# neggles/neurosis

Hardware: AMD Instinct MI355X
Metric: train images/sec (node) SDXL 1024^2 (higher is better)
Workload: dtype bf16

## Files before the change

include/neurosis_hip.h:

```cpp
#ifndef NEUROSIS_HIP_H
#define NEUROSIS_HIP_H

#ifdef __cplusplus
extern "C" {
#endif

const char* nk_last_error(void);
int nk_abi_version(void);

int nk_linear_fwd(const void* x, const void* w, const float* bias, const void* residual, void* y,
                  int M, int N, int K, long ldx, long ldw, long ldr, long ldy, float alpha, void* stream);
int nk_linear_dgrad(const void* dy, const void* w, const void* dx_add, void* dx, int M, int N, int K,
                    long lddy, long ldw, long ldadd, long lddx, void* stream);
long nk_linear_fwd_geglu_ok(int M, int I, int K);
int nk_linear_fwd_geglu(const void* x, const void* w, const float* bias, void* u, void* h, int M, int I, int K, long ldx, long ldw, long ldu,
                        long ldh, void* stream);
int nk_linear_dgrad_geglu(const void* dy, const void* w, const void* u, void* du, int M, int N, int I, long lddy, long ldw, long ldu,
                          long lddu, void* stream);
int nk_linear_fwd_geglu_s(const void* x, const void* w, const float* bias, void* s, void* h, int M, int I, int K, long ldx, long ldw, long lds,
                          long ldh, void* stream);
int nk_linear_dgrad_geglu_s(const void* dy, const void* w, const void* s, void* du, int M, int N, int I, long lddy, long ldw, long lds,
                            long lddu, void* stream);
int nk_linear_wgrad(const void* dy, const void* x, float* dw, int M, int N, int K, long lddy, long ldx,
                    long lddw, int accumulate, void* stream);
// ... 15 lines not shown

int nk_linear_fwd_batched(const void* const* x, const void* const* w, void* const* y, int count, int M, int N, int K,
                          long ldx, long ldw, long ldy, void* stream);

int nk_linear_wgrad_batched(const void* const* dy, const void* const* x, float* const* dw, float* const* dbias, int count, int M, int N,
                            int K, long lddy, long ldx, long lddw, int accumulate, void* stream);

typedef struct NkConvDesc {
  int N, H, W, Cin;
  int Cout, KH, KW;
  int stride;
  int pad_t, pad_l;
  int Ho, Wo;
  int upsample;
} NkConvDesc;
int nk_conv2d_fwd(const NkConvDesc* d, const void* x, const void* w, const float* bias, const void* rowvec,
                  const void* residual, void* y, void* stream);
long nk_conv2d_stats_tiles(const NkConvDesc* d, int stats_groups);
int nk_conv2d_fwd_stats(const NkConvDesc* d, const void* x, const void* w, const float* bias, const void* rowvec, const void* residual,
                        void* y, float* stats_part, int stats_groups, void* stream);
int nk_conv3x3_few_channels_fwd(const void* x, const void* w, const float* bias, void* y, int N, int H, int W, int Cout, int cin_real,
                                void* stream);
int nk_conv_weight_flip(const void* w, void* wt, int Cout, int Cin, int taps, void* stream);
long nk_conv2d_dgrad_flipped_ok(const NkConvDesc* d);
int nk_conv2d_dgrad_flipped(const NkConvDesc* d, const void* dy, const void* wt, void* dx, void* stream);
int nk_conv2d_dgrad(const NkConvDesc* d, const void* dy, const void* w, void* dx, void* stream);
int nk_conv2d_wgrad(const NkConvDesc* d, const void* dy, const void* x, float* dw, int accumulate, void* stream);
int nk_conv2d_wgrad_bias(const NkConvDesc* d, const void* dy, const void* x, float* dw, float* dbias, int accumulate, void* stream);

typedef struct NkAttnDesc {
// ... 229 lines not shown
```

neurosis_amd/csrc/elementwise.hip:

```cpp
#include "../../include/neurosis_hip.h"
#include "nk_common.h"
#include "nk_ew.h"
#include "nk_reduce.h"
#include "norm_plan.h"

struct GegluFwd {
  const bf16_t* u; bf16_t* y; int I;
  __device__ void operator()(long, long row, int ch) const {
    float a[8], g[8];
    ew_load(u + row * 2 * I + ch * 8, a);
    ew_load(u + row * 2 * I + I + ch * 8, g);
#pragma unroll
    for (int e = 0; e < 8; ++e) a[e] *= gelu_erf(g[e]);
    ew_store(y + row * I + ch * 8, a);
  }
};
struct GegluBwd {
  const bf16_t *dy, *u; bf16_t* du; int I;
  __device__ void operator()(long, long row, int ch) const {
    float a[8], g[8], d[8], da[8], dg[8];
    ew_load(u + row * 2 * I + ch * 8, a);
    ew_load(u + row * 2 * I + I + ch * 8, g);
    ew_load(dy + row * I + ch * 8, d);
#pragma unroll
// ... 419 lines not shown
  const int tflip = taps - 1 - tap;
#pragma unroll
  for (int it = 0; it < 2; ++it) {
    const int idx = tid + 256 * it;
    const int r = idx >> 3, ch = idx & 7;
    if (ci0 + r < Cin && co0 + ch * 8 < Cout)
      *(uint4_t*)(wt + ((long)(ci0 + r) * taps + tflip) * Cout + co0 + ch * 8) = *(const uint4_t*)&tile[r][ch * 8];
  }
}
extern "C" int nk_conv_weight_flip(const void* w, void* wt, int Cout, int Cin, int taps, void* stream) {
  NK_CHECK_ARG(w && wt && Cout > 0 && Cin > 0 && taps > 0 && taps <= 65535);
  NK_CHECK_ARG((Cout & 7) == 0 && (Cin & 7) == 0);
  hipLaunchKernelGGL(conv_weight_flip_kernel, dim3((Cin + 63) / 64, (Cout + 63) / 64, taps), dim3(256), 0, (hipStream_t)stream, (const bf16_t*)w, (bf16_t*)wt,
                     Cout, Cin, taps);
  return nk_check_launch("conv_weight_flip_kernel");
}

__global__ __launch_bounds__(256) void conv3x3_few_channels_kernel(const bf16_t* __restrict__ x, const bf16_t* __restrict__ w, const float* __restrict__ bias,
                                                                   bf16_t* __restrict__ y, int N, int H, int W, int Cout, int groups_per_wave) {
  const int lane = threadIdx.x & 63, wave = threadIdx.x >> 6;
  const int r = lane & 15, g = lane >> 4;
  const int co_base = blockIdx.y * 128;
  bf16x8_t wf[8][2];
#pragma unroll
  for (int b = 0; b < 8; ++b) {
    const int co = co_base + b * 16 + r;
    uint2_t t0 = {0u, 0u}, t1 = {0u, 0u}, t8 = {0u, 0u};
    if (co < Cout) {
      t0 = *(const uint2_t*)(w + ((long)co * 9 + 2 * g) * 8);
      t1 = *(const uint2_t*)(w + ((long)co * 9 + 2 * g + 1) * 8);
// ... 508 lines not shown
```

neurosis_amd/csrc/gemm.hip:

```cpp
#include "nk_common.h"
#include "nk_gemm.h"
#include "gemm_plan.h"

#define NTHREADS 256
#define KC_IMAGE_BYTES (128 * 128)
#define MC_ROW_BYTES (128 * 2 + 16)
#define MC_IMAGE_BYTES (BK * MC_ROW_BYTES)
#define OPND_BYTES MC_IMAGE_BYTES
#define STAGE_BYTES (2 * OPND_BYTES)
#define SMEM_BYTES (2 * STAGE_BYTES)

static_assert(SMEM_BYTES >= BM * CS_LD * 4, "epilogue staging must fit");

__device__ __forceinline__ bool is_kc(int mode) { return mode == OP_KC || mode == OP_KCG; }

__device__ __forceinline__ long gather_offset(const NkGather& g, int n, int bh, int bw, int kh, int kw,
                                              int c, bool& valid) {
  int hn = bh + kh * g.ks;
  int wn = bw + kw * g.ks;
  bool ok = (hn >= 0) & (wn >= 0);
  ok &= (((hn | wn) & g.need_even) == 0);
  const int sh = g.div >> 1;
  int h = hn >> sh, w = wn >> sh;
  ok &= (h < g.H) & (w < g.W);
// ... 94 lines not shown
        float v = cs[row * CS_LD + col] * p.alpha;
        float* dst = C + (long)m * p.ldc + n;
        if (p.accumulate) unsafeAtomicAdd(dst, v);
        else *dst = v;
      }
    }
  } else {
    bf16_t* C = (bf16_t*)(p.nbatch ? p.Cb[blockIdx.z] : p.C);
    const bool vec = (p.N & 7) == 0;
#pragma unroll 2
    for (int it = 0; it < (TBM * BN / 8) / TNT; ++it) {
      int idx = tid + it * TNT;
      int row = idx >> 4, cc = idx & 15;
      int m = m0 + row, n = n0 + cc * 8;
      if (m >= p.M || n >= p.N) continue;
      float v[8];
      const float4_t c0 = *(const float4_t*)(cs + row * CS_LD + cc * 8);
      const float4_t c1 = *(const float4_t*)(cs + row * CS_LD + cc * 8 + 4);
      v[0] = c0[0]; v[1] = c0[1]; v[2] = c0[2]; v[3] = c0[3];
      v[4] = c1[0]; v[5] = c1[1]; v[6] = c1[2]; v[7] = c1[3];
      if (p.alpha != 1.0f) {
#pragma unroll
        for (int e = 0; e < 8; ++e) v[e] *= p.alpha;
      }
      if (vec) {
        if (p.bias) {
          const float4_t b0 = *(const float4_t*)(p.bias + n);
          const float4_t b1 = *(const float4_t*)(p.bias + n + 4);
          v[0] += b0[0]; v[1] += b0[1]; v[2] += b0[2]; v[3] += b0[3];
          v[4] += b1[0]; v[5] += b1[1]; v[6] += b1[2]; v[7] += b1[3];
        }
        if (p.rowvec) {
          unsigned b = fdiv((unsigned)m, p.fRowsPerBatch);
          float t[8];
          unpack8(*(const uint4_t*)(p.rowvec + (long)b * p.ld_rowvec + n), t);
#pragma unroll
          for (int e = 0; e < 8; ++e) v[e] += t[e];
        }
        if (p.residual) {
          float t[8];
          unpack8(*(const uint4_t*)(p.residual + (long)m * p.ldr + n), t);
#pragma unroll
          for (int e = 0; e < 8; ++e) v[e] += t[e];
        }
        *(uint4_t*)(C + (long)m * p.ldc + n) = pack8(v);
      } else {
        for (int e = 0; e < 8 && n + e < p.N; ++e) {
          float x = v[e];
          if (p.bias) x += p.bias[n + e];
          if (p.rowvec) x += bf2f(p.rowvec[(long)fdiv((unsigned)m, p.fRowsPerBatch) * p.ld_rowvec + n + e]);
          if (p.residual) x += bf2f(p.residual[(long)m * p.ldr + n + e]);
          C[(long)m * p.ldc + n + e] = f2bf(x);
        }
      }
    }
  }
}

__device__ __attribute__((aligned(64))) unsigned int nk_zero_page[16];

typedef __attribute__((address_space(1))) const void* nk_gptr;
typedef __attribute__((address_space(3))) void* nk_lptr;

__device__ __forceinline__ int mc_swz(int k) { return ((k & 3) | (((k >> 3) & 1) << 2)) << 1; }

template <int MODE, int NP = 4>
struct OperandDMA {
  const bf16_t* P;
  long ld;
  int R, r0, wave, lane;
  int pn[NP], pbh[NP], pbw[NP];
  int tkh0, tkh1, tkw0, tkw1, tc0, tc1;
  bool rvalid[NP < 2 ? 2 : NP];

  __device__ __forceinline__ int kc_row(int i) const { return wave * (NP * 8) + i * 8 + (lane >> 3); }
  __device__ __forceinline__ int kc_chunk() const { return (lane & 7) ^ (lane >> 3); }
  __device__ __forceinline__ int mc_k(int i) const { return (wave * NP + i) * 4 + (lane >> 4); }
  __device__ __forceinline__ int mc_var(int i) const { return (((wave * NP + i) * 4) >> 3) & 1; }
  __device__ __forceinline__ bool mc_valid(int v) const { return v ? rvalid[1] : rvalid[0]; }
  __device__ __forceinline__ int sel(int a0, int a1, int v) const { return v ? a1 : a0; }
  __device__ __forceinline__ int mc_chunk(int v) const { return (lane & 15) ^ (((lane >> 4) | (v << 2)) << 1); }

  __device__ __forceinline__ void init(const bf16_t* p, long ld_, int R_, int r0_, int tid, const NkGather& g) {
    P = p; ld = ld_; R = R_; r0 = r0_; wave = tid >> 6; lane = tid & 63;
    if constexpr (MODE == OP_KC || MODE == OP_KCG) {
#pragma unroll
      for (int i = 0; i < NP; ++i) {
        int r = r0 + kc_row(i);
        rvalid[i] = r < R;
        if constexpr (MODE == OP_KCG) {
          unsigned p_ = rvalid[i] ? (unsigned)r : 0u;
          unsigned n = fdiv(p_, g.fHoWo);
          unsigned rem = p_ - n * g.fHoWo.d;
          unsigned ph = fdiv(rem, g.fWo);
          unsigned pw = rem - ph * g.fWo.d;
          pn[i] = (int)n;
          pbh[i] = (int)ph * g.rs + g.off_h;
          pbw[i] = (int)pw * g.rs + g.off_w;
          if (g.div == 1 && (g.C & 63) == 0) pn[i] = ((pn[i] * g.H + pbh[i]) * g.W + pbw[i]) * g.C + kc_chunk() * 8;
        }
      }
    } else {
#pragma unroll
      for (int v = 0; v < 2; ++v) {
        int r = r0 + mc_chunk(v) * 8;
        rvalid[v] = r < R;
        if constexpr (MODE == OP_MCG) {
          unsigned rr = rvalid[v] ? (unsigned)r : 0u;
          unsigned tap = fdiv(rr, g.fC);
          const int c_ = (int)(rr - tap * g.fC.d);
          unsigned kh = fdiv(tap, g.fKW);
          const int kw_ = (int)(tap - kh * g.fKW.d);
          if (v == 0) { tc0 = c_; tkh0 = (int)kh; tkw0 = kw_; }
// ... 257 lines not shown
  const int per_group = GMv * ntn;
  const int group = wg / per_group;
  const int first_m = group * GMv;
  const int gm = min(GMv, ntm - first_m);
  const int in_group = wg - group * per_group;
  const int nt = in_group / gm;
  const int mt = first_m + (in_group - nt * gm);
  const int m0 = mt * BM, n0 = nt * BN;

  const int kbeg = blockIdx.y * p.ksplit_len;
  const int kend = min(p.K, kbeg + p.ksplit_len);
  const int nk = (kend - kbeg + BK - 1) / BK;

  OperandDMA<AMODE, NP> opa;
  OperandDMA<BMODE, NP> opb;
  opa.init(p.nbatch ? p.Ab[blockIdx.z] : p.A, p.lda, p.M, m0, tid, p.ga);
  opb.init(p.nbatch ? p.Bb[blockIdx.z] : p.B, p.ldb, p.N, n0, tid, p.gb);

  float4_t acc[4][NJ];
#pragma unroll
  for (int i = 0; i < 4; ++i)
#pragma unroll
    for (int j = 0; j < NJ; ++j) acc[i][j] = (float4_t){0.f, 0.f, 0.f, 0.f};
  constexpr bool CAN_BIAS = AMODE == OP_MC && OUT_F32 == 1;
  constexpr int NWN = NW == 4 ? 2 : 4, BPW = 4 / NWN;
  float* const dbias = CAN_BIAS ? (p.nbatch ? p.dbias_b[blockIdx.z] : p.dbias) : nullptr;
  const bool do_bias = CAN_BIAS && dbias != nullptr && nt == 0;
  const int wn_s = __builtin_amdgcn_readfirstlane(wn);
  float4_t accb[BPW];
#pragma unroll
  for (int u = 0; u < BPW; ++u) accb[u] = (float4_t){0.f, 0.f, 0.f, 0.f};
// ... 982 lines not shown
  if (amode == OP_MC) NK_CHECK_ARG((p.M & 7) == 0 && (p.lda & 7) == 0);
  if (bmode == OP_MC) NK_CHECK_ARG((p.N & 7) == 0 && (p.ldb & 7) == 0);
  if (bmode == OP_MCT) NK_CHECK_ARG((p.N & 7) == 0 && (p.tw.co_stride & 7) == 0 && (p.tw.tap_stride & 7) == 0);
  if (bmode == OP_MCG) NK_CHECK_ARG((p.gb.C & 7) == 0);
  if (p.residual) NK_CHECK_ARG(((uintptr_t)p.residual & 15) == 0 && ((p.ldr & 7) == 0 || (p.N & 7) != 0));
  if (!out_f32) NK_CHECK_ARG((p.ldc & 7) == 0 || (p.N & 7) != 0);
  if (p.fRowsPerBatch.d == 0) p.fRowsPerBatch = make_fastdiv(1);

  if (p.dbias || (p.nbatch && p.dbias_b[0])) NK_CHECK_ARG(amode == OP_MC && out_f32);
  if (p.geglu_h) {
    NK_CHECK_ARG(amode == OP_KC && bmode == OP_KC && !out_f32 && !p.nbatch && (p.N & 255) == 0 && (p.ld_h & 7) == 0 && !p.rowvec && !p.residual && p.alpha == 1.0f);
    NK_CHECK_ARG(((uintptr_t)p.geglu_h & 15) == 0 && (!p.bias || ((uintptr_t)p.bias & 15) == 0));
  } else if (p.geglu_u) {
    NK_CHECK_ARG(amode == OP_KC && bmode == OP_MC && !out_f32 && !p.nbatch && (p.N & 7) == 0 && (p.ld_u & 7) == 0 && !p.bias && !p.rowvec && !p.residual);
  }

  const TileEnv env = tile_env();
  const NkGemmPlan pl = nk_gemm_plan(p, amode, bmode, out_f32, allow_splitk, env);
  if (pl.err) {
    nk_set_error(__FILE__, __LINE__, pl.err);
    return NK_ERR_ARG;
  }
  if (pl.zero_c) NK_CHECK_ARG(p.ldc == p.N);
  const int logging = nk_launch_log_mode();
  char line[192];
  if (logging) nk_plan_line(pl, line, sizeof(line));
  if (logging == 3) {
    nk_launch_log_add(pl.name, line);
    return NK_OK;
  }
// ... 54 lines not shown
```

neurosis_amd/csrc/gemm_plan.h:

```cpp
#pragma once
#include "nk_gemm.h"
#include <stdio.h>
#include <stdlib.h>

enum { OP_KC = 0, OP_KCG = 1, OP_MC = 2, OP_MCT = 3, OP_MCG = 4 };

#define BM 128
#define BN 128
#define BK 64
#define GROUP_M 8
#define CS_LD 132
#define V2_OPND_BYTES 16384
#define V2_STAGE_BYTES (2 * V2_OPND_BYTES)
#define V2_SMEM_BYTES (BM * CS_LD * 4)
#define RING_NS 4
#define RING_SMEM_BYTES (RING_NS * V2_STAGE_BYTES)
#define SK_NT 512
#define SK_SMEM_BYTES (2 * V2_STAGE_BYTES)
#define SK_MAX_GRID 512
#define R64_NS 8
#define R64_OPND 8192
#define R64_STAGE (2 * R64_OPND)
#define R64_SMEM (R64_NS * R64_STAGE)
#define XL_BM 256
// ... 302 lines not shown

  if (p.geglu_h) {
    if (amode != OP_KC || !use_xl(env, p, amode, bmode, out_f32, 1)) {
      pl.err = "fused GEGLU forward on a shape the 256 x 256 kernel does not take (ask nk_linear_fwd_geglu_ok first)";
      return pl;
    }
    plan_split(pl, p, 1);
    plan_xl(pl, env, p, OP_KC);
    return pl;
  }
  if (p.geglu_u) {
    plan_split(pl, p, 1);
    plan_ring_or_dma(pl, env, p);
    return pl;
  }
  if (use_halo(env, p, amode, bmode, out_f32)) {
    const NkGather& g = p.ga;
    pl.bn = halo_bn(p.N); pl.halo_rows = halo_tile_rows(p); pl.flag = p.stats_part != nullptr;
    pl.tiles_per_image = cdiv(g.W, CH_TW) * cdiv(g.H, pl.halo_rows);
    plan_kernel(pl, NK_FAM_HALO, halo_name(pl.bn, pl.halo_rows, pl.flag), (long)p.halo_nb * pl.tiles_per_image * (p.N / pl.bn), 1, 1,
                halo_threads(pl.bn), halo_smem(pl.bn, pl.halo_rows));
    pl.k_rotate = k_rotate_on(env, g.C);
    return pl;
  }
  if (use_wgrad_halo(env, p, amode, bmode, out_f32)) {
    int per = 0;
    const int S = wgrad_halo_splits(p, per);
    const long nblk = (long)((p.M + WH_BCO - 1) / WH_BCO) * (p.gb.C / WH_BCI);
    pl.flag = p.dbias != nullptr;
    plan_kernel(pl, NK_FAM_WGRAD_HALO, pl.flag ? "nk_conv3x3_wgrad_halo_kernel<bias=1>" : "nk_conv3x3_wgrad_halo_kernel<bias=0>", nblk * S, 1, 1, 512, WH_SMEM);
// ... 61 lines not shown
```

neurosis_amd/csrc/nk_gemm.h:

```cpp
#pragma once
#include "nk_common.h"

struct NkGather {
  int H, W, C;
  int Ho, Wo;
  int KW;
  int rs, ks;
  int off_h, off_w;
  int div;
  int need_even;
  FastDiv fWo, fHoWo, fC, fKW;
};

struct NkTapW {
  long co_stride, tap_stride;
  FastDiv fCout;
};

struct NkGemmParams {
  const bf16_t* A;
  const bf16_t* B;
  long lda, ldb;
  int M, N, K;
  NkGather ga, gb;
// ... 18 lines not shown
  const bf16_t* Bb[8];
  void* Cb[8];
  unsigned* sk_flags;
  float* sk_ws;
  unsigned* sk_health;
  float* dbias;
  float* dbias_b[8];
  const bf16_t* geglu_u;
  long ld_u;
  bf16_t* geglu_h;
  long ld_h;
  int geglu_save;
  int halo_nb;
  float* stats_part;
  int stats_groups;
};
#define NK_MAX_BATCH 8

enum { NK_OP_KC = 0, NK_OP_KCG = 1, NK_OP_MC = 2, NK_OP_MCT = 3, NK_OP_MCG = 4 };

int nk_gemm_dispatch(NkGemmParams& p, int amode, int bmode, int out_f32, int allow_splitk, hipStream_t stream);
int nk_halo_tiles_per_image(const NkGemmParams& p, int* bn);
int nk_geglu_fwd_fusable(const NkGemmParams& p);
```

neurosis_amd/csrc/ops_gemm.hip:

```cpp
#include "../../include/neurosis_hip.h"
#include "nk_gemm.h"
#include <string.h>

static NkGemmParams zero_params() {
  NkGemmParams p;
  memset(&p, 0, sizeof(p));
  p.alpha = 1.0f;
  p.fRowsPerBatch = make_fastdiv(1);
  p.ga.fWo = p.ga.fHoWo = p.ga.fC = p.ga.fKW = make_fastdiv(1);
  p.gb.fWo = p.gb.fHoWo = p.gb.fC = p.gb.fKW = make_fastdiv(1);
  p.tw.fCout = make_fastdiv(1);
  return p;
}

extern "C" int nk_linear_fwd(const void* x, const void* w, const float* bias, const void* residual, void* y,
                             int M, int N, int K, long ldx, long ldw, long ldr, long ldy, float alpha,
                             void* stream) {
  NkGemmParams p = zero_params();
  p.A = (const bf16_t*)x; p.lda = ldx;
  p.B = (const bf16_t*)w; p.ldb = ldw;
  p.M = M; p.N = N; p.K = K;
  p.C = y; p.ldc = ldy;
  p.bias = bias;
  p.residual = (const bf16_t*)residual; p.ldr = ldr;
// ... 115 lines not shown
  for (int i = 0; i < count; ++i) {
    p.Ab[i] = (const bf16_t*)dy[i];
    p.Bb[i] = (const bf16_t*)x[i];
    p.Cb[i] = dw[i];
    p.dbias_b[i] = dbias ? dbias[i] : nullptr;
  }
  p.A = p.Ab[0]; p.B = p.Bb[0]; p.C = p.Cb[0];
  return nk_gemm_dispatch(p, NK_OP_MC, NK_OP_MC, 1, lddw == K, (hipStream_t)stream);
}

static int check_conv(const NkConvDesc* d) {
  NK_CHECK_ARG(d != nullptr);
  NK_CHECK_ARG(d->N > 0 && d->H > 0 && d->W > 0 && d->Cin > 0 && d->Cout > 0);
  NK_CHECK_ARG(d->KH > 0 && d->KW > 0 && (d->stride == 1 || d->stride == 2 || d->stride == 4));
  NK_CHECK_ARG((d->Cin & 7) == 0 && (d->Cout & 7) == 0);
  NK_CHECK_ARG(!(d->upsample && d->stride != 1));
  const int Hin = d->upsample ? 2 * d->H : d->H, Win = d->upsample ? 2 * d->W : d->W;
  NK_CHECK_ARG(d->Ho > 0 && d->Wo > 0);
  NK_CHECK_ARG((d->Ho - 1) * d->stride - d->pad_t < Hin && (d->Wo - 1) * d->stride - d->pad_l < Win);
  NK_CHECK_ARG((long)d->N * Hin * Win * (long)d->Cin < (1l << 31) && (long)d->N * d->Ho * d->Wo * (long)d->Cout < (1l << 31));
  return NK_OK;
}

static NkGather fwd_gather(const NkConvDesc* d) {
  NkGather g;
  memset(&g, 0, sizeof(g));
  g.H = d->H; g.W = d->W; g.C = d->Cin;
  g.Ho = d->Ho; g.Wo = d->Wo; g.KW = d->KW;
  g.rs = d->stride; g.ks = 1;
  g.off_h = -d->pad_t; g.off_w = -d->pad_l;
  g.div = d->upsample ? 2 : 1;
// ... 7 lines not shown
                                    const void* residual, void* y) {
  NkGemmParams p = zero_params();
  p.A = (const bf16_t*)x;
  p.ga = fwd_gather(d);
  p.B = (const bf16_t*)w; p.ldb = (long)d->KH * d->KW * d->Cin;
  p.M = d->N * d->Ho * d->Wo; p.N = d->Cout; p.K = d->KH * d->KW * d->Cin;
  p.C = y; p.ldc = d->Cout;
  p.bias = bias;
  p.rowvec = (const bf16_t*)rowvec; p.ld_rowvec = d->Cout;
  p.fRowsPerBatch = make_fastdiv(d->Ho * d->Wo);
  p.residual = (const bf16_t*)residual; p.ldr = d->Cout;
  p.halo_nb = (d->KH == 3 && d->KW == 3) ? d->N : 0;
  return p;
}

extern "C" int nk_conv2d_fwd(const NkConvDesc* d, const void* x, const void* w, const float* bias,
                             const void* rowvec, const void* residual, void* y, void* stream) {
  if (int e = check_conv(d)) return e;
  NkGemmParams p = conv_fwd_params(d, x, w, bias, rowvec, residual, y);
  return nk_gemm_dispatch(p, NK_OP_KCG, NK_OP_KC, 0, 0, (hipStream_t)stream);
}

extern "C" long nk_conv2d_stats_tiles(const NkConvDesc* d, int stats_groups) {
  if (check_conv(d)) return 0;
  if (stats_groups < 0 || stats_groups > 32) return 0;
  NkGemmParams p = conv_fwd_params(d, nullptr, nullptr, nullptr, nullptr, nullptr, nullptr);
  int bn = 0;
  const int tiles = nk_halo_tiles_per_image(p, &bn);
  if (tiles && stats_groups) {
    if (d->Cout % stats_groups) return 0;
    if (bn % (d->Cout / stats_groups)) return 0;
  }
  return tiles;
}

extern "C" int nk_conv2d_fwd_stats(const NkConvDesc* d, const void* x, const void* w, const float* bias, const void* rowvec,
                                   const void* residual, void* y, float* stats_part, int stats_groups, void* stream) {
  if (int e = check_conv(d)) return e;
  NK_CHECK_ARG(stats_part && stats_groups > 0);
  NK_CHECK_ARG(nk_conv2d_stats_tiles(d, stats_groups) > 0);
  NkGemmParams p = conv_fwd_params(d, x, w, bias, rowvec, residual, y);
  p.stats_part = stats_part; p.stats_groups = stats_groups;
  return nk_gemm_dispatch(p, NK_OP_KCG, NK_OP_KC, 0, 0, (hipStream_t)stream);
}

extern "C" int nk_conv2d_dgrad(const NkConvDesc* d, const void* dy, const void* w, void* dx, void* stream) {
  if (int e = check_conv(d)) return e;
  const int Hin = d->upsample ? 2 * d->H : d->H, Win = d->upsample ? 2 * d->W : d->W;
  NkGemmParams p = zero_params();
  NkGather g;
  memset(&g, 0, sizeof(g));
  g.H = d->Ho; g.W = d->Wo; g.C = d->Cout;
  g.Ho = Hin; g.Wo = Win; g.KW = d->KW;
  g.rs = 1; g.ks = -1;
  g.off_h = d->pad_t; g.off_w = d->pad_l;
  g.div = d->stride; g.need_even = d->stride - 1;
  g.fWo = make_fastdiv(Win); g.fHoWo = make_fastdiv(Hin * Win);
  g.fC = make_fastdiv(d->Cout); g.fKW = make_fastdiv(d->KW);
  p.A = (const bf16_t*)dy; p.ga = g;
  p.B = (const bf16_t*)w;
  p.tw.co_stride = (long)d->KH * d->KW * d->Cin;
  p.tw.tap_stride = d->Cin;
  p.tw.fCout = make_fastdiv(d->Cout);
  p.M = d->N * Hin * Win; p.N = d->Cin; p.K = d->KH * d->KW * d->Cout;
  p.C = dx; p.ldc = d->Cin;
  return nk_gemm_dispatch(p, NK_OP_KCG, NK_OP_MCT, 0, 0, (hipStream_t)stream);
}

extern "C" long nk_conv2d_dgrad_flipped_ok(const NkConvDesc* d) {
  if (check_conv(d) || d->KH != 3 || d->KW != 3 || d->stride != 1 || d->pad_t != 1 || d->pad_l != 1) return 0;
  const int Hin = d->upsample ? 2 * d->H : d->H, Win = d->upsample ? 2 * d->W : d->W;
  if (d->Ho != Hin || d->Wo != Win) return 0;
  NkConvDesc t = *d;
  t.H = Hin; t.W = Win; t.Cin = d->Cout; t.Cout = d->Cin; t.upsample = 0;
  NkGemmParams p = conv_fwd_params(&t, nullptr, nullptr, nullptr, nullptr, nullptr, nullptr);
  return nk_halo_tiles_per_image(p, nullptr) > 0;
}

extern "C" int nk_conv2d_dgrad_flipped(const NkConvDesc* d, const void* dy, const void* wt, void* dx, void* stream) {
  NK_CHECK_ARG(nk_conv2d_dgrad_flipped_ok(d) == 1);
  const int Hin = d->upsample ? 2 * d->H : d->H, Win = d->upsample ? 2 * d->W : d->W;
  NkConvDesc t = *d;
  t.H = Hin; t.W = Win; t.Cin = d->Cout; t.Cout = d->Cin; t.upsample = 0;
  NkGemmParams p = conv_fwd_params(&t, dy, wt, nullptr, nullptr, nullptr, dx);
  return nk_gemm_dispatch(p, NK_OP_KCG, NK_OP_KC, 0, 0, (hipStream_t)stream);
}

static int conv_wgrad(const NkConvDesc* d, const void* dy, const void* x, float* dw, float* dbias, int accumulate, void* stream) {
  if (int e = check_conv(d)) return e;
  NkGemmParams p = zero_params();
  p.A = (const bf16_t*)dy; p.lda = d->Cout;
  p.B = (const bf16_t*)x; p.gb = fwd_gather(d);
  p.M = d->Cout; p.N = d->KH * d->KW * d->Cin; p.K = d->N * d->Ho * d->Wo;
  p.C = dw; p.ldc = p.N;
  p.accumulate = accumulate;
  p.dbias = dbias;
  p.halo_nb = (d->KH == 3 && d->KW == 3) ? d->N : 0;
  return nk_gemm_dispatch(p, NK_OP_MC, NK_OP_MCG, 1, 1, (hipStream_t)stream);
}
extern "C" int nk_conv2d_wgrad(const NkConvDesc* d, const void* dy, const void* x, float* dw, int accumulate,
                               void* stream) {
  return conv_wgrad(d, dy, x, dw, nullptr, accumulate, stream);
}
extern "C" int nk_conv2d_wgrad_bias(const NkConvDesc* d, const void* dy, const void* x, float* dw, float* dbias, int accumulate,
// ... 5 lines not shown
```

neurosis_amd/lib.py:

```python
from __future__ import annotations

import ctypes as C
import os
from pathlib import Path

import torch

CSRC = Path(__file__).resolve().parent / "csrc"
LIB_PATH = CSRC / "libneurosis_hip.so"

vp, i32, i64, f32 = C.c_void_p, C.c_int, C.c_long, C.c_float


class NkConvDesc(C.Structure):
    _fields_ = [(n, i32) for n in ("N", "H", "W", "Cin", "Cout", "KH", "KW", "stride", "pad_t", "pad_l", "Ho", "Wo", "upsample")]


class NkAttnDesc(C.Structure):
    _fields_ = (
        [(n, i32) for n in ("B", "H", "Lq", "Lk", "D")]
        + [(n, i64) for n in ("sq", "sk", "sv", "so", "bq", "bk", "bv", "bo", "sdq", "sdk", "sdv", "sdo", "bdq", "bdk", "bdv", "bdo")]
        + [("scale", f32), ("causal", i32)]
    )

# ... 11 lines not shown
SIGNATURES: dict[str, list] = {
    "nk_linear_fwd": [vp, vp, vp, vp, vp, i32, i32, i32, i64, i64, i64, i64, f32, vp],
    "nk_linear_dgrad": [vp, vp, vp, vp, i32, i32, i32, i64, i64, i64, i64, vp],
    "nk_linear_dgrad_geglu": [vp, vp, vp, vp, i32, i32, i32, i64, i64, i64, i64, vp],
    "nk_linear_fwd_geglu": [vp, vp, vp, vp, vp, i32, i32, i32, i64, i64, i64, i64, vp],
    "nk_linear_fwd_geglu_s": [vp, vp, vp, vp, vp, i32, i32, i32, i64, i64, i64, i64, vp],
    "nk_linear_dgrad_geglu_s": [vp, vp, vp, vp, i32, i32, i32, i64, i64, i64, i64, vp],
    "nk_linear_wgrad": [vp, vp, vp, i32, i32, i32, i64, i64, i64, i32, vp],
    "nk_linear_fwd_batched": [C.POINTER(vp), C.POINTER(vp), C.POINTER(vp), i32, i32, i32, i32, i64, i64, i64, vp],
    "nk_linear_wgrad_batched": [C.POINTER(vp), C.POINTER(vp), C.POINTER(vp), C.POINTER(vp), i32, i32, i32, i32, i64, i64, i64, i32, vp],
    "nk_linear_wgrad_bias": [vp, vp, vp, vp, i32, i32, i32, i64, i64, i64, i32, vp],
    "nk_conv2d_wgrad_bias": [cdp, vp, vp, vp, vp, i32, vp],
    "nk_conv2d_fwd": [cdp, vp, vp, vp, vp, vp, vp, vp],
    "nk_conv2d_fwd_stats": [cdp, vp, vp, vp, vp, vp, vp, vp, i32, vp],
    "nk_conv_weight_flip": [vp, vp, i32, i32, i32, vp],
    "nk_conv3x3_few_channels_fwd": [vp, vp, vp, vp, i32, i32, i32, i32, i32, vp],
    "nk_conv2d_dgrad": [cdp, vp, vp, vp, vp],
    "nk_conv2d_dgrad_flipped": [cdp, vp, vp, vp, vp],
    "nk_conv2d_wgrad": [cdp, vp, vp, vp, i32, vp],
    "nk_attention_fwd": [adp, vp, vp, vp, vp, vp, vp],
    "nk_attention_bwd": [adp, vp, vp, vp, vp, vp, vp, vp, vp, vp, vp, vp],
    "nk_attention_bwd_causal": [adp, vp, vp, vp, vp, vp, vp, vp, vp, vp, vp],
    "nk_attention_relbias_fwd": [adp, vp, vp, vp, vp, vp, vp],
    "nk_softmax_rows": [vp, i64, i32, vp],
    "nk_softmax_rows_bwd": [vp, vp, i64, i32, f32, vp],
    "nk_groupnorm_fwd": [vp, vp, vp, vp, vp, vp, vp, i32, i32, i32, i32, f32, i32, vp],
    "nk_groupnorm_sums": [vp, vp, vp, i32, i32, i32, i32, vp],
    "nk_groupnorm_sums_from_parts": [vp, vp, vp, i32, i32, i32, vp],
    "nk_groupnorm_apply": [vp, vp, vp, vp, vp, vp, vp, i32, i32, i32, i32, f32, i32, vp],
    "nk_groupnorm_bwd": [vp, vp, vp, vp, vp, vp, vp, vp, vp, vp, vp, i32, i32, i32, i32, i32, i32, vp],
# ... 77 lines not shown
    "nk_debug_launch_log": [i32],
    "nk_health_clear": [],
    "nk_health_export": [vp, vp],
    "nk_health_import": [vp, vp],
    "nk_adafactor_init": [vp, vp],
    "nk_adafactor_chunk": [vp, vp],
    "nk_came_chunk": [vp, vp],
    "nk_adamw8bit_step": [vp, vp],
}

SIZE_QUERIES: dict[str, list] = {
    "nk_groupnorm_ws_floats": [i32, i32, i32, i32],
    "nk_groupnorm_sums_ws_floats": [i32, i32, i32],
    "nk_conv2d_stats_tiles": [cdp, i32],
    "nk_conv2d_dgrad_flipped_ok": [cdp],
    "nk_linear_fwd_geglu_ok": [i32, i32, i32],
    "nk_layernorm_ws_floats": [i32, i32],
    "nk_layernorm_part_rows": [i32],
    "nk_colsum_ws_floats": [i64, i32],
    "nk_batchnorm_ws_floats": [i64, i32],
    "nk_lpips_layer_ws_floats": [i32, i32],
    "nk_attention_bwd_ws_floats": [adp],
    "nk_vq_search_ws_floats": [i64, i32],
    "nk_vq_quantize_ws_floats": [i64],
    "nk_gumbel_softmax_ws_floats": [i64],
    "nk_resample_ws_floats": [i64, i32, i32, i32, i32],
    "nk_adafactor_tensor_bytes": [],
    "nk_came_tensor_bytes": [],
    "nk_adamw8bit_tensor_bytes": [],
    "nk_gemm_sk_status": [],
# ... 60 lines not shown
```

neurosis_amd/models/diffusion.py:

```python
from __future__ import annotations

import os
from contextlib import contextmanager, nullcontext
from math import ceil
from typing import Callable, Optional

import torch
from torch import Tensor, nn

from .. import ops
from ..modules.diffusion import Denoiser, DiffusionLoss, OpenAIWrapper, UNetModel
from ..nn import FlatParamStore
from .autoencoder import AutoencoderKL


class PrecomputedConditioner(nn.Module):

    def forward(self, batch: dict, force_zero_embeddings=None) -> dict:
        zeroed = set(force_zero_embeddings or ())
        out = {}
        for k in ("crossattn", "vector", "concat"):
            if k in batch and batch[k] is not None:
                out[k] = torch.zeros_like(batch[k]) if k in zeroed else batch[k]
        return out
# ... 87 lines not shown
            raise NotImplementedError("stream_optimizer (the update streamed block by block behind backward) does not drive the text towers' groups")
        import torch.distributed as dist

        if dist.is_available() and dist.is_initialized() and dist.get_world_size() > 1:
            raise NotImplementedError("trainable text towers at world size > 1: their gradient exchange is not built (one GPU only)")

    def setup_flat_params(self) -> FlatParamStore:
        self._check_trainable_embedders()
        self.store = FlatParamStore([p for p in self.model.diffusion_model.parameters() if p.requires_grad])
        self.embedder_stores = []
        for e in self.trainable_embedders():
            st = FlatParamStore(e.trained_parameters())
            st.state.assume_zeroed = False
            self.embedder_stores.append(st)
        self.store.state.assume_zeroed = False
        if self.store.master.is_cuda:
            self.store.state.wgrad_stream = torch.cuda.Stream(device=self.store.master.device)
        if self.use_ema:
            self.configure_ema(self.ema_decay_rate)
        if self.optimizer is not None and self._torch_optimizer is None:
            self.configure_optimizers()
        self.stream_optimizer = self.stream_optimizer
        return self.store

    @property
    def stream_optimizer(self) -> bool:
        return self._stream_optimizer

    @stream_optimizer.setter
    def stream_optimizer(self, on: bool) -> None:
# ... 306 lines not shown
```

neurosis_amd/ops.py:

```python
from __future__ import annotations

import ctypes as C
import math
import os
import threading
import weakref
from dataclasses import dataclass
from typing import Callable, Optional

import torch
from torch import Tensor

from . import lib
from .lib import NkAttnDesc, NkConvDesc, call, query

BF16 = torch.bfloat16


class EngineState:

    _live = weakref.WeakSet()

    def __init__(self, wgrad_stream=None):
        self.grad_accumulate = False
        self.assume_zeroed = False
        self.wgrad_stream = wgrad_stream
        self.batch_wgrads = os.environ.get("NK_BATCH_WGRADS", "1") != "0"
        self.norm_params_on_side_stream: Optional[bool] = None
        self.deferred: Optional[list] = None
        self.segment_hook: Optional[Callable] = None
        EngineState._live.add(self)

    def derived(self) -> "EngineState":
        return EngineState(self.wgrad_stream)


_capture_depth = 0


def capturing() -> bool:
    return _capture_depth > 0


class capture_scope:
    def __enter__(self):
# ... 432 lines not shown
                raise ValueError(f"linear bwd: geglu_u must be [{M}, {2 * K}], got {tuple(geglu_u.shape)}")
            du = torch.empty(M, 2 * K, dtype=BF16, device=dy.device)
            wq = w2d(weight)
            call(entry, dy.data_ptr(), wq.data_ptr(), geglu_u.data_ptr(), du.data_ptr(), M, N, K, dy.stride(0), wq.stride(0),
                 geglu_u.stride(0), du.stride(0), _stream())
            return du
        return gemm_nn(dy, w2d(weight), dx_add)

    return bwd


def _conv_desc(N, H, W, Cin, Cout, KH, KW, stride, pad_t, pad_l, Ho, Wo, upsample) -> NkConvDesc:
    return NkConvDesc(N, H, W, Cin, Cout, KH, KW, stride, pad_t, pad_l, Ho, Wo, int(upsample))


def groupnorm_sums(x: Img, groups: int) -> Tensor:
    if x.sums is not None and x.sums.shape == (x.N, 2 * groups):
        return x.sums
    sums = torch.empty(x.N, 2 * groups, dtype=torch.float32, device=x.t.device)
    ws = _ws(query("nk_groupnorm_ws_floats", x.N, x.H * x.W, x.C, groups), x.t.device)
    call("nk_groupnorm_sums", x.t.data_ptr(), sums.data_ptr(), ws.data_ptr(), x.N, x.H * x.W, x.C, groups, _stream())
    return sums


def conv2d_fwd(x: Img, weight: Tensor, bias: Optional[Tensor], stride: int = 1, padding=1, upsample: bool = False,
               rowvec: Optional[Tensor] = None, residual: Optional[Tensor] = None, need_dx: bool = True,
               asym_pad: bool = False, stats_groups: Optional[int] = None, cin_real: Optional[int] = None):
    Cout, Cin, KH, KW = weight.shape
    if x.C != Cin:
        raise ValueError(f"conv2d: input has {x.C} channels, weight expects {Cin}")
# ... 1 lines not shown
    if asym_pad:
        pad_t = pad_l = 0
        Ho = (Hin + 1 - KH) // stride + 1
        Wo = (Win + 1 - KW) // stride + 1
    else:
        pad_t = pad_l = int(padding)
        Ho = (Hin + 2 * pad_t - KH) // stride + 1
        Wo = (Win + 2 * pad_l - KW) // stride + 1
    d = _conv_desc(x.N, x.H, x.W, Cin, Cout, KH, KW, stride, pad_t, pad_l, Ho, Wo, upsample)
    y = torch.empty(x.N * Ho * Wo, Cout, dtype=BF16, device=x.t.device)
    _check2d(x.t, "x")
    if not x.t.is_contiguous():
        raise ValueError("conv2d: x must be dense channels-last")
    tiles = query("nk_conv2d_stats_tiles", C.byref(d), stats_groups) if stats_groups else 0
    sums_out = None
    if tiles:
        dev = x.t.device
        part = torch.empty(x.N, tiles, 2 * stats_groups, dtype=torch.float32, device=dev)
        call("nk_conv2d_fwd_stats", C.byref(d), x.t.data_ptr(), w2d(weight).data_ptr(), _p(bias), _p(rowvec), _p(residual), y.data_ptr(),
             part.data_ptr(), stats_groups, _stream())
        sums_out = torch.empty(x.N, 2 * stats_groups, dtype=torch.float32, device=dev)
        ws = _ws(query("nk_groupnorm_sums_ws_floats", x.N, tiles, stats_groups), dev)
        call("nk_groupnorm_sums_from_parts", part.data_ptr(), sums_out.data_ptr(), ws.data_ptr(), x.N, tiles, stats_groups, _stream())
    elif (cin_real in (3, 4) and Cin == 8 and KH == 3 and KW == 3 and stride == 1 and pad_t == 1 and not asym_pad and not upsample and rowvec is None
          and residual is None and Cout % 8 == 0):
        call("nk_conv3x3_few_channels_fwd", x.t.data_ptr(), w2d(weight).data_ptr(), _p(bias), y.data_ptr(), x.N, x.H, x.W, Cout, cin_real, _stream())
    else:
        call("nk_conv2d_fwd", C.byref(d), x.t.data_ptr(), w2d(weight).data_ptr(), _p(bias), _p(rowvec), _p(residual), y.data_ptr(), _stream())
    out = Img(y, x.N, Ho, Wo, sums_out)

    def bwd(dy: Tensor):
        _check2d(dy, "dy")
        if not dy.is_contiguous():
            raise ValueError("conv2d bwd: dy must be dense")
        acc = state_of(weight).grad_accumulate

        if weight.requires_grad:
            if bias is not None:
                on_wgrad_stream(lambda: call("nk_conv2d_wgrad_bias", C.byref(d), dy.data_ptr(), x.t.data_ptr(), g2d(weight).data_ptr(), grad_flat(bias).data_ptr(),
                                             wgrad_mode(weight), _stream()), dy, x.t, owner=weight)
            else:
                on_wgrad_stream(lambda: call("nk_conv2d_wgrad", C.byref(d), dy.data_ptr(), x.t.data_ptr(), g2d(weight).data_ptr(), wgrad_mode(weight), _stream()),
                                dy, x.t, owner=weight)
        drow = None
        if rowvec is not None:
            drow32 = torch.empty(x.N, Cout, dtype=torch.float32, device=dy.device)
            ws = _ws(x.N * query("nk_colsum_ws_floats", Ho * Wo, Cout), dy.device)
            call("nk_colsum_batched", dy.data_ptr(), drow32.data_ptr(), ws.data_ptr(), Ho * Wo, Cout, dy.stride(0), x.N, 0, _stream())
            drow = cast_bf16(drow32)
        dx = None
# ... 1020 lines not shown
```

Before: 26.37.

## Fold nearest-upsample into 3x3 conv as four 2x2 sub-pixel phase GEMMs

For a nearest-neighbour 2x upsample followed by a 3x3 conv, the weights are pre-folded into four 2x2 phase kernels. The forward then runs as a batched implicit GEMM over the low-resolution input, with each phase writing interleaved output rows. This uses about 4/9 of the MACs and skips the upsampled gather. Backward dgrad runs as a stride-2 4x4 conv on dy, and wgrad computes the folded-weight gradient and unfolds it back to 3x3. The costs are an extra fold kernel (cached per weight stamp), an fp32 scratch buffer plus an unfold kernel for wgrad, and a separate bias colsum.

```diff
diff --git a/include/neurosis_hip.h b/include/neurosis_hip.h
--- a/include/neurosis_hip.h
+++ b/include/neurosis_hip.h
@@ -53,6 +53,9 @@
   int Ho, Wo;
   int upsample;
 } NkConvDesc;
+long nk_conv2d_up_phase_ok(const NkConvDesc* d);
+int nk_conv_up_fold(const void* w, void* vf, void* v, int Cout, int Cin, void* stream);
+int nk_conv_up_unfold(const float* dvt, float* dw, int Cout, int Cin, int accumulate, void* stream);
 int nk_conv2d_fwd(const NkConvDesc* d, const void* x, const void* w, const float* bias, const void* rowvec,
                   const void* residual, void* y, void* stream);
 long nk_conv2d_stats_tiles(const NkConvDesc* d, int stats_groups);
diff --git a/neurosis_amd/csrc/elementwise.hip b/neurosis_amd/csrc/elementwise.hip
--- a/neurosis_amd/csrc/elementwise.hip
+++ b/neurosis_amd/csrc/elementwise.hip
@@ -457,6 +457,86 @@
   hipLaunchKernelGGL(conv_weight_flip_kernel, dim3((Cin + 63) / 64, (Cout + 63) / 64, taps), dim3(256), 0, (hipStream_t)stream, (const bf16_t*)w, (bf16_t*)wt,
                      Cout, Cin, taps);
   return nk_check_launch("conv_weight_flip_kernel");
+}
+
+__global__ __launch_bounds__(256) void conv_up_fold_kernel(const bf16_t* __restrict__ w, bf16_t* __restrict__ vf, bf16_t* __restrict__ v, int Cout, int Cin) {
+  const int cpr = Cin >> 3;
+  const long idx = (long)blockIdx.x * 256 + threadIdx.x;
+  if (idx >= (long)Cout * cpr) return;
+  const int co = (int)(idx / cpr), ci = (int)(idx - (long)co * cpr) * 8;
+  float t[3][3][8];
+#pragma unroll
+  for (int k = 0; k < 9; ++k) unpack8(*(const uint4_t*)(w + ((long)co * 9 + k) * Cin + ci), t[k / 3][k % 3]);
+  float r[4][3][8];
+#pragma unroll
+  for (int kw = 0; kw < 3; ++kw)
+#pragma unroll
+    for (int e = 0; e < 8; ++e) {
+      r[0][kw][e] = t[2][kw][e];
+      r[1][kw][e] = t[1][kw][e] + t[2][kw][e];
+      r[2][kw][e] = t[0][kw][e] + t[1][kw][e];
+      r[3][kw][e] = t[0][kw][e];
+    }
+#pragma unroll
+  for (int u = 0; u < 4; ++u)
+#pragma unroll
+    for (int x = 0; x < 4; ++x) {
+      float s[8];
+#pragma unroll
+      for (int e = 0; e < 8; ++e) s[e] = x == 0 ? r[u][2][e] : x == 1 ? r[u][1][e] + r[u][2][e] : x == 2 ? r[u][0][e] + r[u][1][e] : r[u][0][e];
+      const uint4_t o = pack8(s);
+      *(uint4_t*)(v + ((long)co * 16 + u * 4 + x) * Cin + ci) = o;
+      const int a = (3 - u) & 1, p = (3 - u) >> 1, b = (3 - x) & 1, q = (3 - x) >> 1;
+      *(uint4_t*)(vf + ((long)co * 16 + (a * 2 + b) * 4 + p * 2 + q) * Cin + ci) = o;
+    }
+}
+extern "C" int nk_conv_up_fold(const void* w, void* vf, void* v, int Cout, int Cin, void* stream) {
+  NK_CHECK_ARG(w && vf && v && Cout > 0 && Cin > 0 && (Cin & 7) == 0);
+  NK_CHECK_ARG(nk_aligned16(w) && nk_aligned16(vf) && nk_aligned16(v));
+  const long n = (long)Cout * (Cin >> 3);
+  hipLaunchKernelGGL(conv_up_fold_kernel, dim3((unsigned)((n + 255) / 256)), dim3(256), 0, (hipStream_t)stream, (const bf16_t*)w, (bf16_t*)vf, (bf16_t*)v, Cout, Cin);
+  return nk_check_launch("conv_up_fold_kernel");
+}
+
+__global__ __launch_bounds__(256) void conv_up_unfold_kernel(const float* __restrict__ dvt, float* __restrict__ dw, int Cout, int Cin, int accumulate) {
+  __shared__ float tile[9][32][33];
+  const int ci0 = blockIdx.x * 32, co0 = blockIdx.y * 32;
+  const int tx = threadIdx.x & 31, ty = threadIdx.x >> 5;
+  for (int yy = ty; yy < 32; yy += 8) {
+    const int ci = ci0 + yy, co = co0 + tx;
+    float g[4][4];
+#pragma unroll
+    for (int k = 0; k < 16; ++k) g[k >> 2][k & 3] = (ci < Cin && co < Cout) ? dvt[((long)ci * 16 + k) * Cout + co] : 0.f;
+    float r[3][4];
+#pragma unroll
+    for (int x = 0; x < 4; ++x) {
+      r[0][x] = g[2][x] + g[3][x];
+      r[1][x] = g[1][x] + g[2][x];
+      r[2][x] = g[0][x] + g[1][x];
+    }
+#pragma unroll
+    for (int kh = 0; kh < 3; ++kh) {
+      tile[kh * 3 + 0][yy][tx] = r[kh][2] + r[kh][3];
+      tile[kh * 3 + 1][yy][tx] = r[kh][1] + r[kh][2];
+      tile[kh * 3 + 2][yy][tx] = r[kh][0] + r[kh][1];
+    }
+  }
+  __syncthreads();
+  for (int yy = ty; yy < 32; yy += 8) {
+    const int co = co0 + yy, ci = ci0 + tx;
+    if (co >= Cout || ci >= Cin) continue;
+#pragma unroll
+    for (int k = 0; k < 9; ++k) {
+      float* dst = dw + ((long)co * 9 + k) * Cin + ci;
+      const float s = tile[k][tx][yy];
+      *dst = accumulate ? *dst + s : s;
+    }
+  }
+}
+extern "C" int nk_conv_up_unfold(const float* dvt, float* dw, int Cout, int Cin, int accumulate, void* stream) {
+  NK_CHECK_ARG(dvt && dw && Cout > 0 && Cin > 0 && (accumulate == 0 || accumulate == 1));
+  hipLaunchKernelGGL(conv_up_unfold_kernel, dim3((Cin + 31) / 32, (Cout + 31) / 32), dim3(256), 0, (hipStream_t)stream, dvt, dw, Cout, Cin, accumulate);
+  return nk_check_launch("conv_up_unfold_kernel");
 }
 
 __global__ __launch_bounds__(256) void conv3x3_few_channels_kernel(const bf16_t* __restrict__ x, const bf16_t* __restrict__ w, const float* __restrict__ bias,
diff --git a/neurosis_amd/csrc/gemm.hip b/neurosis_amd/csrc/gemm.hip
--- a/neurosis_amd/csrc/gemm.hip
+++ b/neurosis_amd/csrc/gemm.hip
@@ -132,6 +132,7 @@
       int row = idx >> 4, cc = idx & 15;
       int m = m0 + row, n = n0 + cc * 8;
       if (m >= p.M || n >= p.N) continue;
+      const long mo = p.up_phase ? 2l * m + 2l * p.up_W * fdiv((unsigned)m, p.fUpW) + (long)(blockIdx.z >> 1) * 2 * p.up_W + (blockIdx.z & 1) : (long)m;
       float v[8];
       const float4_t c0 = *(const float4_t*)(cs + row * CS_LD + cc * 8);
       const float4_t c1 = *(const float4_t*)(cs + row * CS_LD + cc * 8 + 4);
@@ -161,14 +162,14 @@
 #pragma unroll
           for (int e = 0; e < 8; ++e) v[e] += t[e];
         }
-        *(uint4_t*)(C + (long)m * p.ldc + n) = pack8(v);
+        *(uint4_t*)(C + mo * p.ldc + n) = pack8(v);
       } else {
         for (int e = 0; e < 8 && n + e < p.N; ++e) {
           float x = v[e];
           if (p.bias) x += p.bias[n + e];
           if (p.rowvec) x += bf2f(p.rowvec[(long)fdiv((unsigned)m, p.fRowsPerBatch) * p.ld_rowvec + n + e]);
           if (p.residual) x += bf2f(p.residual[(long)m * p.ldr + n + e]);
-          C[(long)m * p.ldc + n + e] = f2bf(x);
+          C[mo * p.ldc + n + e] = f2bf(x);
         }
       }
     }
@@ -199,7 +200,7 @@
   __device__ __forceinline__ int sel(int a0, int a1, int v) const { return v ? a1 : a0; }
   __device__ __forceinline__ int mc_chunk(int v) const { return (lane & 15) ^ (((lane >> 4) | (v << 2)) << 1); }
 
-  __device__ __forceinline__ void init(const bf16_t* p, long ld_, int R_, int r0_, int tid, const NkGather& g) {
+  __device__ __forceinline__ void init(const bf16_t* p, long ld_, int R_, int r0_, int tid, const NkGather& g, int oh = 0, int ow = 0) {
     P = p; ld = ld_; R = R_; r0 = r0_; wave = tid >> 6; lane = tid & 63;
     if constexpr (MODE == OP_KC || MODE == OP_KCG) {
 #pragma unroll
@@ -213,8 +214,8 @@
           unsigned ph = fdiv(rem, g.fWo);
           unsigned pw = rem - ph * g.fWo.d;
           pn[i] = (int)n;
-          pbh[i] = (int)ph * g.rs + g.off_h;
-          pbw[i] = (int)pw * g.rs + g.off_w;
+          pbh[i] = (int)ph * g.rs + g.off_h + oh;
+          pbw[i] = (int)pw * g.rs + g.off_w + ow;
           if (g.div == 1 && (g.C & 63) == 0) pn[i] = ((pn[i] * g.H + pbh[i]) * g.W + pbw[i]) * g.C + kc_chunk() * 8;
         }
       }
@@ -502,7 +503,8 @@
 
   OperandDMA<AMODE, NP> opa;
   OperandDMA<BMODE, NP> opb;
-  opa.init(p.nbatch ? p.Ab[blockIdx.z] : p.A, p.lda, p.M, m0, tid, p.ga);
+  if constexpr (AMODE == OP_KCG) opa.init(p.nbatch ? p.Ab[blockIdx.z] : p.A, p.lda, p.M, m0, tid, p.ga, p.up_phase ? (int)(blockIdx.z >> 1) : 0, p.up_phase ? (int)(blockIdx.z & 1) : 0);
+  else opa.init(p.nbatch ? p.Ab[blockIdx.z] : p.A, p.lda, p.M, m0, tid, p.ga);
   opb.init(p.nbatch ? p.Bb[blockIdx.z] : p.B, p.ldb, p.N, n0, tid, p.gb);
 
   float4_t acc[4][NJ];
@@ -1515,6 +1517,10 @@
   } else if (p.geglu_u) {
     NK_CHECK_ARG(amode == OP_KC && bmode == OP_MC && !out_f32 && !p.nbatch && (p.N & 7) == 0 && (p.ld_u & 7) == 0 && !p.bias && !p.rowvec && !p.residual);
   }
+  if (p.up_phase) {
+    NK_CHECK_ARG(amode == OP_KCG && bmode == OP_KC && !out_f32 && p.nbatch == 4 && p.ga.div == 1 && (p.ga.C & 63) == 0 && p.up_W == p.ga.Wo && p.fUpW.d == (unsigned)p.up_W);
+    NK_CHECK_ARG(!p.rowvec && !p.residual && !p.stats_part && !p.geglu_u && !p.geglu_h && (long)p.M * 4 * p.ldc < (1l << 40));
+  }
 
   const TileEnv env = tile_env();
   const NkGemmPlan pl = nk_gemm_plan(p, amode, bmode, out_f32, allow_splitk, env);
diff --git a/neurosis_amd/csrc/gemm_plan.h b/neurosis_amd/csrc/gemm_plan.h
--- a/neurosis_amd/csrc/gemm_plan.h
+++ b/neurosis_amd/csrc/gemm_plan.h
@@ -340,6 +340,12 @@
     plan_ring_or_dma(pl, env, p);
     return pl;
   }
+  if (p.up_phase) {
+    plan_split(pl, p, 1);
+    plan_ring_or_dma(pl, env, p);
+    if (pl.family != NK_FAM_DMA) pl.err = "phase launch of an upsample convolution outside the 128 x 128 double-buffer kernel";
+    return pl;
+  }
   if (use_halo(env, p, amode, bmode, out_f32)) {
     const NkGather& g = p.ga;
     pl.bn = halo_bn(p.N); pl.halo_rows = halo_tile_rows(p); pl.flag = p.stats_part != nullptr;
diff --git a/neurosis_amd/csrc/nk_gemm.h b/neurosis_amd/csrc/nk_gemm.h
--- a/neurosis_amd/csrc/nk_gemm.h
+++ b/neurosis_amd/csrc/nk_gemm.h
@@ -56,6 +56,9 @@
   int halo_nb;
   float* stats_part;
   int stats_groups;
+  int up_phase;
+  int up_W;
+  FastDiv fUpW;
 };
 #define NK_MAX_BATCH 8
 
diff --git a/neurosis_amd/csrc/ops_gemm.hip b/neurosis_amd/csrc/ops_gemm.hip
--- a/neurosis_amd/csrc/ops_gemm.hip
+++ b/neurosis_amd/csrc/ops_gemm.hip
@@ -153,7 +153,9 @@
   NK_CHECK_ARG(d->N > 0 && d->H > 0 && d->W > 0 && d->Cin > 0 && d->Cout > 0);
   NK_CHECK_ARG(d->KH > 0 && d->KW > 0 && (d->stride == 1 || d->stride == 2 || d->stride == 4));
   NK_CHECK_ARG((d->Cin & 7) == 0 && (d->Cout & 7) == 0);
-  NK_CHECK_ARG(!(d->upsample && d->stride != 1));
+  NK_CHECK_ARG(d->upsample >= 0 && d->upsample <= 2 && !(d->upsample && d->stride != 1));
+  if (d->upsample == 2)
+    NK_CHECK_ARG(d->KH == 3 && d->KW == 3 && d->pad_t == 1 && d->pad_l == 1 && d->Ho == 2 * d->H && d->Wo == 2 * d->W && (d->Cin & 63) == 0);
   const int Hin = d->upsample ? 2 * d->H : d->H, Win = d->upsample ? 2 * d->W : d->W;
   NK_CHECK_ARG(d->Ho > 0 && d->Wo > 0);
   NK_CHECK_ARG((d->Ho - 1) * d->stride - d->pad_t < Hin && (d->Wo - 1) * d->stride - d->pad_l < Win);
@@ -191,9 +193,55 @@
   return p;
 }
 
+static NkConvDesc up_transposed_desc(const NkConvDesc* d) {
+  NkConvDesc t = *d;
+  t.H = 2 * d->H; t.W = 2 * d->W; t.Cin = d->Cout; t.Cout = d->Cin;
+  t.KH = t.KW = 4; t.stride = 2; t.pad_t = t.pad_l = 1; t.Ho = d->H; t.Wo = d->W; t.upsample = 0;
+  return t;
+}
+
+extern "C" long nk_conv2d_up_phase_ok(const NkConvDesc* d) {
+  if (!d || !d->upsample) return 0;
+  NkConvDesc u = *d;
+  u.upsample = 2;
+  const long rows = (long)d->N * d->H * d->W;
+  return check_conv(&u) == NK_OK && rows * 4 * d->Cout < (1l << 31) ? 1 : 0;
+}
+
+static int up_phase_fwd(const NkConvDesc* d, const void* x, const void* vf, const float* bias, void* y, hipStream_t stream) {
+  NkGemmParams p = zero_params();
+  NkGather g;
+  memset(&g, 0, sizeof(g));
+  g.H = d->H; g.W = d->W; g.C = d->Cin;
+  g.Ho = d->H; g.Wo = d->W; g.KW = 2;
+  g.rs = 1; g.ks = 1;
+  g.off_h = -1; g.off_w = -1;
+  g.div = 1;
+  g.fWo = make_fastdiv(d->W); g.fHoWo = make_fastdiv(d->H * d->W);
+  g.fC = make_fastdiv(d->Cin); g.fKW = make_fastdiv(2);
+  p.ga = g;
+  p.M = d->N * d->H * d->W; p.N = d->Cout; p.K = 4 * d->Cin;
+  p.ldb = 16l * d->Cin;
+  p.ldc = d->Cout;
+  p.bias = bias;
+  p.nbatch = 4;
+  for (int z = 0; z < 4; ++z) {
+    p.Ab[z] = (const bf16_t*)x;
+    p.Bb[z] = (const bf16_t*)vf + (long)z * 4 * d->Cin;
+    p.Cb[z] = y;
+  }
+  p.A = p.Ab[0]; p.B = p.Bb[0]; p.C = y;
+  p.up_phase = 1; p.up_W = d->W; p.fUpW = make_fastdiv(d->W);
+  return nk_gemm_dispatch(p, NK_OP_KCG, NK_OP_KC, 0, 0, stream);
+}
+
 extern "C" int nk_conv2d_fwd(const NkConvDesc* d, const void* x, const void* w, const float* bias,
                              const void* rowvec, const void* residual, void* y, void* stream) {
   if (int e = check_conv(d)) return e;
+  if (d->upsample == 2) {
+    NK_CHECK_ARG(!rowvec && !residual);
+    return up_phase_fwd(d, x, w, bias, y, (hipStream_t)stream);
+  }
   NkGemmParams p = conv_fwd_params(d, x, w, bias, rowvec, residual, y);
   return nk_gemm_dispatch(p, NK_OP_KCG, NK_OP_KC, 0, 0, (hipStream_t)stream);
 }
@@ -223,6 +271,19 @@
 
 extern "C" int nk_conv2d_dgrad(const NkConvDesc* d, const void* dy, const void* w, void* dx, void* stream) {
   if (int e = check_conv(d)) return e;
+  if (d->upsample == 2) {
+    const NkConvDesc t = up_transposed_desc(d);
+    if (int e = check_conv(&t)) return e;
+    NkGemmParams p = zero_params();
+    p.A = (const bf16_t*)dy; p.ga = fwd_gather(&t);
+    p.B = (const bf16_t*)w;
+    p.tw.co_stride = 16l * d->Cin;
+    p.tw.tap_stride = d->Cin;
+    p.tw.fCout = make_fastdiv(d->Cout);
+    p.M = d->N * d->H * d->W; p.N = d->Cin; p.K = 16 * d->Cout;
+    p.C = dx; p.ldc = d->Cin;
+    return nk_gemm_dispatch(p, NK_OP_KCG, NK_OP_MCT, 0, 0, (hipStream_t)stream);
+  }
   const int Hin = d->upsample ? 2 * d->H : d->H, Win = d->upsample ? 2 * d->W : d->W;
   NkGemmParams p = zero_params();
   NkGather g;
@@ -245,7 +306,7 @@
 }
 
 extern "C" long nk_conv2d_dgrad_flipped_ok(const NkConvDesc* d) {
-  if (check_conv(d) || d->KH != 3 || d->KW != 3 || d->stride != 1 || d->pad_t != 1 || d->pad_l != 1) return 0;
+  if (check_conv(d) || d->KH != 3 || d->KW != 3 || d->stride != 1 || d->pad_t != 1 || d->pad_l != 1 || d->upsample == 2) return 0;
   const int Hin = d->upsample ? 2 * d->H : d->H, Win = d->upsample ? 2 * d->W : d->W;
   if (d->Ho != Hin || d->Wo != Win) return 0;
   NkConvDesc t = *d;
@@ -265,6 +326,11 @@
 
 static int conv_wgrad(const NkConvDesc* d, const void* dy, const void* x, float* dw, float* dbias, int accumulate, void* stream) {
   if (int e = check_conv(d)) return e;
+  if (d->upsample == 2) {
+    NK_CHECK_ARG(!dbias && accumulate == 0);
+    const NkConvDesc t = up_transposed_desc(d);
+    return conv_wgrad(&t, x, dy, dw, nullptr, 0, stream);
+  }
   NkGemmParams p = zero_params();
   p.A = (const bf16_t*)dy; p.lda = d->Cout;
   p.B = (const bf16_t*)x; p.gb = fwd_gather(d);
diff --git a/neurosis_amd/lib.py b/neurosis_amd/lib.py
--- a/neurosis_amd/lib.py
+++ b/neurosis_amd/lib.py
@@ -49,6 +49,8 @@
     "nk_conv2d_fwd": [cdp, vp, vp, vp, vp, vp, vp, vp],
     "nk_conv2d_fwd_stats": [cdp, vp, vp, vp, vp, vp, vp, vp, i32, vp],
     "nk_conv_weight_flip": [vp, vp, i32, i32, i32, vp],
+    "nk_conv_up_fold": [vp, vp, vp, i32, i32, vp],
+    "nk_conv_up_unfold": [vp, vp, i32, i32, i32, vp],
     "nk_conv3x3_few_channels_fwd": [vp, vp, vp, vp, i32, i32, i32, i32, i32, vp],
     "nk_conv2d_dgrad": [cdp, vp, vp, vp, vp],
     "nk_conv2d_dgrad_flipped": [cdp, vp, vp, vp, vp],
@@ -156,6 +158,7 @@
     "nk_groupnorm_sums_ws_floats": [i32, i32, i32],
     "nk_conv2d_stats_tiles": [cdp, i32],
     "nk_conv2d_dgrad_flipped_ok": [cdp],
+    "nk_conv2d_up_phase_ok": [cdp],
     "nk_linear_fwd_geglu_ok": [i32, i32, i32],
     "nk_layernorm_ws_floats": [i32, i32],
     "nk_layernorm_part_rows": [i32],
diff --git a/neurosis_amd/models/diffusion.py b/neurosis_amd/models/diffusion.py
--- a/neurosis_amd/models/diffusion.py
+++ b/neurosis_amd/models/diffusion.py
@@ -125,6 +125,7 @@
             st.state.assume_zeroed = False
             self.embedder_stores.append(st)
         self.store.state.assume_zeroed = False
+        self.store.state.up_phase = True
         if self.store.master.is_cuda:
             self.store.state.wgrad_stream = torch.cuda.Stream(device=self.store.master.device)
         if self.use_ema:
diff --git a/neurosis_amd/ops.py b/neurosis_amd/ops.py
--- a/neurosis_amd/ops.py
+++ b/neurosis_amd/ops.py
@@ -29,6 +29,7 @@
         self.norm_params_on_side_stream: Optional[bool] = None
         self.deferred: Optional[list] = None
         self.segment_hook: Optional[Callable] = None
+        self.up_phase = False
         EngineState._live.add(self)
 
     def derived(self) -> "EngineState":
@@ -491,6 +492,30 @@
     return NkConvDesc(N, H, W, Cin, Cout, KH, KW, stride, pad_t, pad_l, Ho, Wo, int(upsample))
 
 
+def up_phase_enabled(weight=None) -> bool:
+    env = os.environ.get("NK_CONV_UP_PHASE")
+    if env is not None:
+        return env != "0"
+    return bool(state_of(weight).up_phase)
+
+
+def conv_up_folded(weight: Tensor):
+    Cout, Cin = weight.shape[0], weight.shape[1]
+    half = 16 * Cout * Cin
+    stamp = _param_stamp(weight)
+    cache = getattr(weight, "_nk_up_fold", None)
+    buf = None
+    if cache is not None and cache[1].device == weight.device and cache[1].numel() == 2 * half:
+        buf = cache[1]
+        if cache[0] == stamp and not capturing():
+            return buf[:half], buf[half:]
+    if buf is None:
+        buf = torch.empty(2 * half, dtype=BF16, device=weight.device)
+    call("nk_conv_up_fold", w2d(weight).data_ptr(), buf.data_ptr(), buf[half:].data_ptr(), Cout, Cin, _stream())
+    weight._nk_up_fold = (stamp, buf)
+    return buf[:half], buf[half:]
+
+
 def groupnorm_sums(x: Img, groups: int) -> Tensor:
     if x.sums is not None and x.sums.shape == (x.N, 2 * groups):
         return x.sums
@@ -522,7 +547,12 @@
         raise ValueError("conv2d: x must be dense channels-last")
     tiles = query("nk_conv2d_stats_tiles", C.byref(d), stats_groups) if stats_groups else 0
     sums_out = None
-    if tiles:
+    phase = bool(upsample and rowvec is None and residual is None and up_phase_enabled(weight) and query("nk_conv2d_up_phase_ok", C.byref(d)))
+    if phase:
+        d = _conv_desc(x.N, x.H, x.W, Cin, Cout, KH, KW, stride, pad_t, pad_l, Ho, Wo, 2)
+        vf, v = conv_up_folded(weight)
+        call("nk_conv2d_fwd", C.byref(d), x.t.data_ptr(), vf.data_ptr(), _p(bias), None, None, y.data_ptr(), _stream())
+    elif tiles:
         dev = x.t.device
         part = torch.empty(x.N, tiles, 2 * stats_groups, dtype=torch.float32, device=dev)
         call("nk_conv2d_fwd_stats", C.byref(d), x.t.data_ptr(), w2d(weight).data_ptr(), _p(bias), _p(rowvec), _p(residual), y.data_ptr(),
@@ -542,6 +572,24 @@
         if not dy.is_contiguous():
             raise ValueError("conv2d bwd: dy must be dense")
         acc = state_of(weight).grad_accumulate
+
+        if phase:
+            if weight.requires_grad:
+                def up_wgrad():
+                    add = wgrad_mode(weight) == 1
+                    dvt = torch.empty(Cin * 16 * Cout, dtype=torch.float32, device=dy.device)
+                    call("nk_conv2d_wgrad", C.byref(d), dy.data_ptr(), x.t.data_ptr(), dvt.data_ptr(), 0, _stream())
+                    call("nk_conv_up_unfold", dvt.data_ptr(), g2d(weight).data_ptr(), Cout, Cin, int(add), _stream())
+                    if bias is not None:
+                        colsum(dy, grad_flat(bias), add)
+
+                on_wgrad_stream(up_wgrad, dy, x.t, owner=weight)
+            dx = None
+            if need_dx:
+                dxt = torch.empty(x.N * x.H * x.W, Cin, dtype=BF16, device=dy.device)
+                call("nk_conv2d_dgrad", C.byref(d), dy.data_ptr(), v.data_ptr(), dxt.data_ptr(), _stream())
+                dx = Img(dxt, x.N, x.H, x.W)
+            return dx, None
 
         if weight.requires_grad:
             if bias is not None:
```

After: 26.62 (median of 6 runs). No clear change (+0.9%).
